# Mark-Rindler/PTRT-game-engine

Hardware: AMD Instinct MI355X
Metric: Mrays/s (higher is better)
Workload: dtype f32

## Files before the change

ptrt-game-engine_amd/csrc/pt_kernels.hip.h:

```cpp
#pragma once
#include "pt_device.hip.h"

namespace pt {

struct Camera {
    f3 origin, llc, horizontal, vertical, u, v, w;
    float lens_radius;
};

struct KParams {
    const float4 *mesh_recs;
    const float4 *nodes;
    const float4 *nodes2;
    const int2 *leaves;
    const float4 *tris;
    const int4 *slot_face;
    const float4 *tlas_nodes;
    const int2 *tlas_leaves;
    const int *tlas_mesh_ids;
    const float4 *tlas_heads;
    float inst_c2;
    const float4 *materials;
    const float4 *lights;
    const float2 *blue_noise;
    const float4 *tlas_root_box;
    int tlas_root_ref;
    int n_meshes, n_lights;
    int stack_entries;
    int pair_meshes;
    int pair_tri_slots;
    int pair_max_leaf;
    int tlas_max_leaf;
    int tlas_depth;
    int tlas_any_rounds;
    int pair_split;
    int steal;
    int csteal;
    int csteal_min;
    int csteal_follow;
    int csteal_leaf_min;
    int leaf_min;
    int leaf_pairs;
    int fetch_min;
    int n_nodes;
    int top_off;
    int n_tiles;
    int lds_extra;
    int lds_flags;
    int pair_cap;
    int lds_wave, lds_wave_bytes;
    Camera cam;
    f3 sky_top, sky_bottom;
    int use_sky;
    const float4 *env;
    int env_w, env_h;
    int width, height;
    int y0, rows;
    int il_period, il_phase;
    int tiles_x;
    int split_n, split_i;
    int spp, max_depth, frame_count;
    int sample_sync;
    int tile_run;
    uint32_t *rng;
    size_t rng_plane;
    float *accum, *normal, *depth;
    int *object_id;
    unsigned char *rgb8;
    int rgb8_frame;
    int ticket_tiles;
    unsigned int *queue;
    unsigned long long *counters;
};
constexpr int COUNTER_WORDS = 4;

PT_DEV int global_row(int yl, int y0, int il_period, int il_phase) {
    return il_period > 1 ? ((((yl >> 3) * il_period + il_phase) << 3) | (yl & 7)) : y0 + yl;
}

PT_DEV int rgb8_row(const KParams &K, int yl) {
    return K.rgb8_frame ? K.height - 1 - global_row(yl, K.y0, K.il_period, K.il_phase) : K.rows - 1 - yl;
}

constexpr int MESH_REC_F4 = 12;
constexpr int NODE2_F4 = 12;
constexpr int TOP_LEVELS = 3;
constexpr int TOP_NODES = (1 << TOP_LEVELS) - 1;
constexpr int TLAS_HEAD_F4 = 7;
// ... 713 lines not shown
```

ptrt-game-engine_amd/csrc/pt_render.hip.h:

```cpp
#pragma once
#include "pt_kernels.hip.h"

namespace pt {

struct CycleAcc;
struct PairLds {
    CycleAcc *cyc;
    int stat_bounce;
    float4 *tris;
    int4 *meshtab;
    float4 *meshbox;
    const float4 *topnodes;
    uint32_t *pairs;
    unsigned long long *best;
    uint32_t *occ;
    uint2 *stack;
    int *leafx;
    uint2 *tstack;
    unsigned long long *lkey;
    unsigned char *owner;
    const float2 *jit;
    const float2 *bn;
    const float4 *lights;
    const float4 *mats;
// ... 49 lines not shown
    char *p = (char *)base;
    const int meshes = K.pair_meshes;
    l.tris = (float4 *)p;
    p += (size_t)K.pair_tri_slots * 48 + (size_t)meshes * PAIR_PAD * 16;
    l.meshtab = (int4 *)p;
    p += (size_t)meshes * 16;
    l.meshbox = (float4 *)p;
    char *x = (char *)base + K.lds_extra;
    l.jit = (const float2 *)x;
    l.lights = (const float4 *)(x + 16 * 8);
    l.mats = l.lights + ((K.lds_flags & 1) ? K.n_lights * 4 : 0);
    char *w = (char *)base + K.lds_wave + wave * K.lds_wave_bytes;
    l.best = (unsigned long long *)w;
    l.occ = (uint32_t *)(w + 256);
    l.pairs = (uint32_t *)(w + 512);
    w += 512 + pm1_pair_bytes(meshes);
    l.bn = (const float2 *)w;
    w += (K.lds_flags & 8) ? 64 * 8 : 0;
    l.count = (unsigned long long *)w;
    return l;
}

PT_DEV size_t shared_lds_bytes(int meshes) { return (size_t)meshes * (32 + TOP_NODES * 64); }
PT_DEV size_t wave_lds_bytes(int meshes, int stack_entries) {
    return 512 + (size_t)meshes * 128 + 256 + (size_t)stack_entries * 512 + LEAF_PAIR_BYTES;
}
PT_DEV PairLds carve_pair_lds_wg(void *base, int wave, int meshes, int stack_entries) {
    PairLds l{};
    char *p = (char *)base;
    l.meshtab = nullptr;
    l.meshbox = (float4 *)p;
    p += (size_t)meshes * 32;
    l.topnodes = (const float4 *)p;
    p += (size_t)meshes * TOP_NODES * 64;
    p += (size_t)wave * wave_lds_bytes(meshes, stack_entries);
    l.best = (unsigned long long *)p;
    p += 512;
    l.pairs = (uint32_t *)p;
    p += (size_t)meshes * 128;
    l.occ = (uint32_t *)p;
    p += 256;
    l.stack = (uint2 *)p;
    p += (size_t)stack_entries * 512;
    l.lkey = (unsigned long long *)p;
    p += 512;
    l.owner = (unsigned char *)p;
    l.tris = nullptr;
    l.tstack = nullptr;
    l.leafx = nullptr;
    return l;
}

__device__ unsigned long long g_trav_bounce[64];
__device__ unsigned long long g_trav_stats[32];
#ifdef PT_MARKS
#define PT_MARK(x) asm volatile("; MARK " x)
#else
#define PT_MARK(x)
#endif
#ifdef PT_TRAV_STATS
struct TravStats {
    unsigned v[8] = {0, 0, 0, 0, 0, 0, 0, 0};
    PT_DEV void wave(int i, int lane) {
        if (lane == __builtin_ctzll(__builtin_amdgcn_ballot_w64(true)))
            ++v[i];
    }
    PT_DEV void lanes(int i) { ++v[i]; }
    PT_DEV void flush(int base, int lane, int bounce = -1) {
        for (int i = 0; i < 8; ++i) {
            unsigned a = v[i];
            for (int off = 32; off > 0; off >>= 1)
                a += __shfl_xor(a, off);
            if (lane == 0 && a) {
                atomicAdd(&g_trav_stats[base + i], (unsigned long long)a);
                if (bounce >= 0)
                    atomicAdd(&g_trav_bounce[(bounce < 3 ? bounce : 3) * 16 + base + i], (unsigned long long)a);
            }
        }
    }
};
__device__ unsigned long long g_trav_dbg[4 * 256 + 1 + 8];
#define TS_DBG(a, b, c, d)                                                                                                \
    do {                                                                                                                 \
        const unsigned long long i_ = atomicAdd(&g_trav_dbg[1024], 1ull);                                                \
        if (i_ < 256) {                                                                                                  \
            g_trav_dbg[4 * i_] = (a);                                                                                    \
            g_trav_dbg[4 * i_ + 1] = (b);                                                                                \
            g_trav_dbg[4 * i_ + 2] = (c);                                                                                \
            g_trav_dbg[4 * i_ + 3] = (d);                                                                                \
        }                                                                                                                \
    } while (0)
#define TS_EVENT(slot) atomicAdd(&g_trav_dbg[1025 + (slot)], 1ull)
#define TS_WAVE(i) ts.wave(i, lane)
#define TS_LANE(i) ts.lanes(i)
struct CycleAcc {
    unsigned long long c[8] = {0, 0, 0, 0, 0, 0, 0, 0};
    PT_DEV void flush(int lane) {
        if (lane == 0)
            for (int i = 0; i < 8; ++i)
                atomicAdd(&g_trav_stats[24 + i], c[i]);
    }
};
#define TS_LANES(slot, cond)                                                                                             \
    do {                                                                                                                 \
        const unsigned long long ts_m = __builtin_amdgcn_ballot_w64(cond);                                               \
        if (lane == __builtin_ctzll(__builtin_amdgcn_ballot_w64(true)))                                                   \
            atomicAdd(&g_trav_stats[slot], (unsigned long long)__builtin_popcountll(ts_m));                                 \
    } while (0)
#define TS_NOW() __builtin_readcyclecounter()
#define TS_ADD(slot, t) (cyc.c[(slot) - 8] += __builtin_readcyclecounter() - (t))
#define TS_ADDL(slot, t) (L.cyc->c[(slot) - 8] += __builtin_readcyclecounter() - (t))
#ifdef PT_TS_SHADING
constexpr bool TS_SHADING = true;
#else
constexpr bool TS_SHADING = false;
#endif
#define TS_ADDQ(slot, t) do { if (!TS_SHADING) TS_ADD(slot, t); } while (0)
#define TS_ADDLQ(slot, t) do { if (!TS_SHADING) TS_ADDL(slot, t); } while (0)
#else
constexpr bool TS_SHADING = false;
#define TS_ADDQ(slot, t) (void)(t)
#define TS_ADDLQ(slot, t) (void)(t)
struct TravStats {
    PT_DEV void flush(int, int, int = -1) {}
};
#define TS_EVENT(slot)
#define TS_DBG(a, b, c, d)
#define TS_WAVE(i)
#define TS_LANE(i)
struct CycleAcc {
    PT_DEV void flush(int) {}
};
#define TS_LANES(slot, cond)
#define TS_NOW() 0ull
#define TS_ADD(slot, t) (void)(t)
#define TS_ADDL(slot, t) (void)(t)
#endif

PT_DEV void wave_lds_order() {
    __builtin_amdgcn_wave_barrier();
    asm volatile("" ::: "memory");
}

PT_DEV void wave_sync() { wave_lds_order(); }

PT_DEV int lane_prefix(unsigned long long mask) {
    return __builtin_amdgcn_mbcnt_hi((uint32_t)(mask >> 32), __builtin_amdgcn_mbcnt_lo((uint32_t)mask, 0u));
}

PT_DEV MeshHead staged_mesh_head(const PairLds &L, int i) {
    const float4 a = L.meshbox[2 * i], b = L.meshbox[2 * i + 1];
    MeshHead h;
    h.bmin = mk3(a.x, a.y, a.z);
    h.bmax = mk3(b.x, b.y, b.z);
    h.root_ref = __builtin_amdgcn_readfirstlane(__float_as_int(a.w));
    const int fm = __builtin_amdgcn_readfirstlane(__float_as_int(b.w));
    h.flags = fm & 0xff;
    h.mesh = fm >> 8;
    return h;
}
PT_DEV int4 staged_mesh_entry(const PairLds &L, int i) {
    const int root = __float_as_int(lds_ld1((const float *)L.meshbox, 8 * i + 3));
    const int fm = __float_as_int(lds_ld1((const float *)L.meshbox, 8 * i + 7));
    return make_int4(root, 0, fm & 0xff, fm >> 8);
}

PT_DEV void leaf_prefix(int cnt, int &start, int &total) {
    int st = 0, tot = 0;
#pragma unroll
    for (int b = 0; b < 5; ++b) {
        const unsigned long long m = __builtin_amdgcn_ballot_w64((cnt >> b) & 1);
        st += lane_prefix(m) << b;
        tot += __builtin_popcountll(m) << b;
    }
    start = st;
    total = tot;
}

template <bool ANY>
PT_DEV int build_pairs(const KParams &K, const PairLds &L, int lane, bool alive, f3 o, f3 d, float tMax) {
    const RayO w = make_ray(o, d);
    float tE;
    alive = alive && slab(tlas_bmin(K), tlas_bmax(K), w, ANY ? tMax : T_FAR, tE);
    if (ANY)
        L.occ[lane] = 0u;
    else
        L.best[lane] = ~0ull;
    int base = 0;
    for (int i = 0; i < K.pair_meshes; ++i) {
        const MeshHead mh = staged_mesh_head(L, i);
        if (ANY && (mh.flags & 2))
            continue;
        bool hb;
        if (mh.flags & 1) {
            float ds;
            const RayO lr = local_ray(K, mh.mesh, w, ds);
            hb = alive && slab(mh.bmin, mh.bmax, lr, ANY ? tMax * ds : T_FAR, tE);
        } else {
            hb = alive && slab(mh.bmin, mh.bmax, w, ANY ? tMax : T_FAR, tE);
        }
        const unsigned long long bal = __builtin_amdgcn_ballot_w64(hb);
        if (hb) {
            ((uint16_t *)L.pairs)[base + lane_prefix(bal)] = (uint16_t)((uint32_t)lane | ((uint32_t)i << 6));
        }
        base += __builtin_popcountll(bal);
    }
    return base;
}

template <int GEN = 0> PT_DEV void pair_ray_from(const KParams &K, const int4 mt, f3 &o, f3 &d, float &dirScale) {
    dirScale = 1.0f;
    if (mt.z & 1) {
        const float4 *rec = GEN ? (K.tlas_heads + mt.w * TLAS_HEAD_F4) : (K.mesh_recs + mt.w * MESH_REC_F4);
        const f3 lo = xform_point(rec[2], rec[3], rec[4], o);
        const f3 ld = xform_dir(rec[2], rec[3], rec[4], d);
        dirScale = length(ld);
        o = lo;
        d = normalize(ld);
    }
}

PT_DEV Hit closest_hit_pairs(const KParams &K, const PairLds &L, int lane, bool alive, f3 o, f3 d, int &order) {
    const int P = build_pairs<false>(K, L, lane, alive, o, d, T_FAR);
    wave_sync();
    for (int c = 0; c < P; c += 64) {
        const int n = (P - c) < 64 ? (P - c) : 64;
        int sh = 0;
        while (K.pair_split && (n << (sh + 1)) <= 64 && (2 << sh) <= K.pair_max_leaf)
            ++sh;
        const int p = c + (lane >> sh), sub = lane & ((1 << sh) - 1);
        const bool valid = (lane >> sh) < n;
        const uint32_t e = ((const uint16_t *)L.pairs)[valid ? p : 0];
        const int r = (int)(e & 63u), oi = (int)(e >> 6);
        const int4 mt = L.meshtab[oi];
        f3 po = mk3(__shfl(o.x, r), __shfl(o.y, r), __shfl(o.z, r));
        f3 pd = mk3(__shfl(d.x, r), __shfl(d.y, r), __shfl(d.z, r));
        float dirScale;
        pair_ray_from<false>(K, mt, po, pd, dirScale);
        RayO pr;
        pr.o = po;
        pr.d = pd;
        float tb = T_FAR;
        int bi = -1;
        const int iters = (K.pair_max_leaf + (1 << sh) - 1) >> sh;
        for (int it = 0; it < iters; ++it) {
            const int i = sub + (it << sh);
            const int slot = mt.x + (i < mt.y ? i : 0);
            const float4 *tp = L.tris + slot * 3 + oi * PAIR_PAD;
            const float4 p0 = tp[0], p1 = tp[1], p2 = tp[2];
            asm volatile("" ::"v"(p0.w), "v"(p1.w), "v"(p2.w));
            float t, u, v;
            const bool ok = tri_test(mk3(p0.x, p0.y, p0.z), mk3(p1.x, p1.y, p1.z), mk3(p2.x, p2.y, p2.z), pr, tb, t, u, v);
            if (ok && i < mt.y) {
                tb = t;
                bi = i;
            }
        }
        if (valid && bi >= 0) {
            const float tw = (mt.z & 1) ? tb / dirScale : tb;
            const unsigned long long key =
                ((unsigned long long)__float_as_uint(tw) << 32) | ((unsigned long long)(uint32_t)oi << 16) | (uint32_t)bi;
            __hip_atomic_fetch_min(&L.best[r], key, __ATOMIC_RELAXED, __HIP_MEMORY_SCOPE_WORKGROUP);
        }
    }
    wave_sync();
    const unsigned long long key = L.best[lane];
    wave_sync();
    Hit h;
    h.u = h.v = 0.0f;
    order = 0;
    if (!alive || key == ~0ull) {
        h.t = h.t_local = T_FAR;
        h.mesh = -1;
        h.slot = -1;
        return h;
    }
    const int oi = (int)((key >> 16) & 0xffffu), bi = (int)(key & 0xffffu);
    order = oi;
    const int4 mt = L.meshtab[oi];
    h.t = __uint_as_float((uint32_t)(key >> 32));
    h.mesh = mt.w;
    h.slot = mt.x + bi;
    h.t_local = h.t;
    if (mt.z & 1) {
        const float4 *rec = K.mesh_recs + mt.w * MESH_REC_F4;
        RayO pr;
        pr.o = xform_point(rec[2], rec[3], rec[4], o);
        pr.d = normalize(xform_dir(rec[2], rec[3], rec[4], d));
        const float4 *tp = L.tris + h.slot * 3 + oi * PAIR_PAD;
        const float4 p0 = tp[0], p1 = tp[1], p2 = tp[2];
        float t, u, v;
        tri_test(mk3(p0.x, p0.y, p0.z), mk3(p1.x, p1.y, p1.z), mk3(p2.x, p2.y, p2.z), pr, T_FAR, t, u, v);
        h.t_local = t;
    }
    return h;
}

PT_DEV bool any_hit_pairs(const KParams &K, const PairLds &L, int lane, bool alive, f3 o, f3 d, float tMax) {
    const int P = build_pairs<true>(K, L, lane, alive, o, d, tMax);
    float *tmaxv = (float *)L.best;
    tmaxv[lane] = tMax;
    wave_sync();
    for (int c = 0; c < P; c += 64) {
        const int n = (P - c) < 64 ? (P - c) : 64;
        int sh = 0;
        while ((n << (sh + 1)) <= 64 && (2 << sh) <= K.pair_max_leaf)
            ++sh;
        const int p = c + (lane >> sh), sub = lane & ((1 << sh) - 1);
        const bool valid = (lane >> sh) < n;
        const uint32_t e = ((const uint16_t *)L.pairs)[valid ? p : 0];
        const int r = (int)(e & 63u), oi = (int)(e >> 6);
        const int4 mt = L.meshtab[oi];
        f3 po = mk3(__shfl(o.x, r), __shfl(o.y, r), __shfl(o.z, r));
        f3 pd = mk3(__shfl(d.x, r), __shfl(d.y, r), __shfl(d.z, r));
        float dirScale;
        pair_ray_from<false>(K, mt, po, pd, dirScale);
        RayO pr;
        pr.o = po;
        pr.d = pd;
        float tm = tmaxv[r];
        if (mt.z & 1)
            tm = tm * dirScale;
        bool found = false;
        const int iters = (K.pair_max_leaf + (1 << sh) - 1) >> sh;
        for (int it = 0; it < iters; ++it) {
            const int i = sub + (it << sh);
            const int slot = mt.x + (i < mt.y ? i : 0);
            const float4 *tp = L.tris + slot * 3 + oi * PAIR_PAD;
            const float4 p0 = tp[0], p1 = tp[1], p2 = tp[2];
            asm volatile("" ::"v"(p0.w), "v"(p1.w), "v"(p2.w));
            float t, u, v;
            const bool ok = tri_test(mk3(p0.x, p0.y, p0.z), mk3(p1.x, p1.y, p1.z), mk3(p2.x, p2.y, p2.z), pr, tm, t, u, v);
            found |= ok && (i < mt.y);
        }
        if (valid && found)
            L.occ[r] = 1u;
    }
    wave_sync();
    const bool occluded = alive && (L.occ[lane] != 0u);
    wave_sync();
    return occluded;
}

template <int GEN> PT_DEV int4 pair_mesh(const KParams &K, const PairLds &L, int r, int order) {
    if (!GEN)
        return staged_mesh_entry(L, order);
    const int j = GEN == 2 ? order : L.leafx[(order & (TLAS_SLOTS - 1)) * 64 + r] + (order >> 2);
    const int root = __float_as_int(K.tlas_heads[TLAS_HEAD_F4 * j].w), flags = __float_as_int(K.tlas_heads[TLAS_HEAD_F4 * j + 1].w);
    return make_int4(root, 0, flags, j);
}

PT_DEV void fetch_node(const KParams &K, const PairLds &L, int cur, int local, int order, float4 &n0, float4 &n1, float4 &n2,
                       float4 &n3) {
    if (L.topnodes && (unsigned)local < (unsigned)TOP_NODES) {
        const float4 *q = L.topnodes + (order * TOP_NODES + local) * 4;
        n0 = q[0];
        n1 = q[1];
        n2 = q[2];
        n3 = q[3];
    } else {
        n0 = K.nodes[cur * 4 + 0];
        n1 = K.nodes[cur * 4 + 1];
        n2 = K.nodes[cur * 4 + 2];
        n3 = K.nodes[cur * 4 + 3];
    }
}

#ifndef PT_TWO_LEVEL
#define PT_TWO_LEVEL 0
#endif
PT_DEV bool descend2(const float4 *__restrict__ nodes2, LdsStack stk, int &sp, const RayO &pr, float tb, int &cur) {
    const float4 *rec = nodes2 + (size_t)cur * NODE2_F4;
    const float4 n0 = rec[0], n1 = rec[1], n2 = rec[2], n3 = rec[3];
    float tL, tR;
    const bool hL = slab(mk3(n0.x, n0.y, n0.z), mk3(n0.w, n1.x, n1.y), pr, tb, tL);
    const bool hR = slab(mk3(n1.z, n1.w, n2.x), mk3(n2.y, n2.z, n2.w), pr, tb, tR);
    if (!(hL || hR))
        return true;
    const bool nearL = hL && (!hR || tL <= tR);
    const int Lr = __float_as_int(n3.x), Rr = __float_as_int(n3.y);
    if (nearL ? hR : hL) {
        stk.push(sp, nearL ? Rr : Lr, nearL ? tR : tL);
        ++sp;
    }
    cur = nearL ? Lr : Rr;
    if (cur < 0)
        return false;
    const float4 *g = rec + (nearL ? 4 : 8);
    const float4 g0 = g[0], g1 = g[1], g2 = g[2], g3 = g[3];
    const bool hGL = slab(mk3(g0.x, g0.y, g0.z), mk3(g0.w, g1.x, g1.y), pr, tb, tL);
    const bool hGR = slab(mk3(g1.z, g1.w, g2.x), mk3(g2.y, g2.z, g2.w), pr, tb, tR);
    if (!(hGL || hGR))
// ... 1299 lines not shown
                rd = normalize(dir);
            } else {
                f3 p;
                do {
                    const float a = rng_uniform(rng);
                    const float b = rng_uniform(rng);
                    p = 2.0f * mk3(a, b, 0.0f) - mk3(1.0f, 1.0f, 0.0f);
                } while (dot(p, p) >= 1.0f);
                const f3 rdisk = KA.cam.lens_radius * p;
                const f3 offset = KA.cam.u * rdisk.x + KA.cam.v * rdisk.y;
                const f3 dir = KA.cam.llc + u * KA.cam.horizontal + v * KA.cam.vertical - KA.cam.origin - offset;
                ro = KA.cam.origin + offset;
                rd = normalize(dir);
            }
            ray_spec = true;
            prev_was_specular = true;
            throughput = mk3(1.0f);
            if (!MERGED)
                acc = mk3(0.0f);
            sb &= 0xffff;
            fresh = false;
        }

        if (PMODE == 1 || TS_SHADING)
            TS_ADD(8, t_pa);
        const bool act = live && !fresh;
#ifdef PT_TRAV_STATS
        {
            const unsigned long long am = __builtin_amdgcn_ballot_w64(act);
            PL.stat_bounce = am ? __builtin_amdgcn_readlane(sb >> 16, __builtin_ctzll(am)) : -1;
        }
#endif
        PT_MARK("B");
        phase_prio<PMODE, 1, 0>();
        const KParams &KB = kparams(kp0);
        Hit h;
        int h_order = 0;
        if (MERGED) {
            bool blocked = false;
            const unsigned long long t_tr = TS_NOW();
            trace_merged(KB, PL, lane, act, ro, rd, pending, park_o, park_d, park_tmax, h, blocked, cyc);
            TS_ADD(12, t_tr);
            if (pending && !blocked)
                acc = acc + pend;
            pending = false;
            if (fin) {
                acc = clamp_vector_soft(acc, 100.0f);
                close_sample(acc);
                acc = mk3(0.0f);
                fin = false;
            }
        } else {
            const unsigned long long t_tr = TS_NOW();
            h = (PMODE == 1)   ? closest_hit_pairs(KB, PL, lane, act, ro, rd, h_order)
                : (PMODE == 2) ? closest_hit_pairs_dyn(KB, PL, lane, act, ro, rd)
                : (PMODE == 3) ? closest_hit_pairs_tlas(KB, PL, lane, act, ro, rd, cyc)
                               : closest_hit<GEOM>(KB, act, ro, rd, stk);
            TS_ADD(12, t_tr);
        }

        PT_MARK("C");
        phase_prio<PMODE, 2, 1>();
        const KParams &KC = kparams(kp0);
        const unsigned long long t_pc = TS_NOW();
        bool end_path = false, shaded = false, want_shadow = false;
        Surface hit;
        hit.point = hit.normal = mk3(0.0f);
        hit.t = 0.0f;
        hit.front_face = true;
        f3 L = mk3(0.0f), light_scale = mk3(0.0f), shadow_o = mk3(0.0f);
        float pdf_sample = 1.0f, shadow_tmax = 0.0f, light_att = 1.0f;
        if (!LDS_COUNT)
            n_ext += (uint32_t)__builtin_popcountll(__builtin_amdgcn_ballot_w64(act));
        if (act) {
            if (h.mesh < 0) {
                if (sb == 0) {
                    const size_t idx = pidx(KC.width);
                    float zero = 0.0f;
                    asm volatile("" : "+v"(zero));
                    KC.normal[idx * 3 + 0] = zero;
                    KC.normal[idx * 3 + 1] = zero;
                    KC.normal[idx * 3 + 2] = zero;
                    KC.depth[idx] = 1e30f;
                    KC.object_id[idx] = -1;
                }
                if (KC.use_sky) {
                    if (KC.env) {
                        const float phi = det_atan2(rd.z, rd.x);
                        const float theta = det_acos(max_(-1.0f, min_(1.0f, rd.y)));
                        const float u = (phi + PI_F) * (1.0f / TWO_PI_F);
                        const float v = theta * (1.0f / PI_F);
                        acc = acc + throughput * tex2d_env(KC.env, KC.env_w, KC.env_h, u, v);
                    } else {
                        const float t = 0.5f * (rd.y + 1.0f);
                        acc = acc + throughput * lerp(KC.sky_bottom, KC.sky_top, t);
                    }
                } else {
                    acc = acc + throughput * mk3(0.0f);
                }
                end_path = true;
            } else {
                shaded = true;
                if (PMODE == 1) {
                    const int ti = (h.slot * 3 + h_order * PAIR_PAD) * 4;
                    const f3 gn = mk3(lds_ld1((const float *)PL.tris, ti + 3), lds_ld1((const float *)PL.tris, ti + 7),
                                      lds_ld1((const float *)PL.tris, ti + 11));
                    const int fl = __float_as_int(lds_ld1((const float *)PL.meshtab, h_order * 4 + 2));
// ... 91 lines not shown
        PT_MARK("C2");
        phase_prio<PMODE, 3, 2>();
        const KParams &KC2 = kparams(kp0);
        const unsigned long long t_pc2 = TS_NOW();
        bool lit = false;
        f3 lit_now = mk3(0.0f);
        if (want_shadow) {
            int mi = mats_lds ? h_order : h.mesh;
            asm volatile("" : "+v"(mi));
            const Material mat = mats_lds ? load_material<true, MAT_F4>(PL.mats, mi) : load_material(KC2.materials, mi);
            const f3 V = -rd;
            const f3 bsdf = evaluateBSDF<FULL>(hit, mat, L, V);
            if (pdf_sample > 0.0f) {
                f3 direct = bsdf * light_scale * light_att / pdf_sample;
                direct = clamp_vector_soft(direct, 500.0f);
                if (direct.x > 0.0f || direct.y > 0.0f || direct.z > 0.0f) {
                    const float pdf_brdf = material_pdf<FULL>(hit, mat, V, L);
                    const float wgt = mis_weight(pdf_sample, pdf_brdf);
                    lit_now = throughput * direct * wgt;
                    lit = true;
                }
            }
        }

        {
            const unsigned long long zm = __builtin_amdgcn_ballot_w64(want_shadow && !lit);
            if (zm) {
                if (LDS_COUNT) {
                    if (lane == 0)
                        __hip_atomic_fetch_add((__attribute__((address_space(3))) unsigned long long *)(lds_count + 1),
                                               (unsigned long long)__builtin_popcountll(zm), __ATOMIC_RELAXED,
                                               __HIP_MEMORY_SCOPE_WORKGROUP);
                } else {
                    n_zero += (uint32_t)__builtin_popcountll(zm);
                }
            }
        }
        if (PMODE == 1 || TS_SHADING)
            TS_ADD(10, t_pc2);
        TS_LANES(21, lit);
        PT_MARK("D");
        phase_prio<PMODE, 4, 3>();
        const KParams &KD = kparams(kp0);
        const unsigned long long t_sh = TS_NOW();
        if (MERGED) {
            if (lit) {
                pend = lit_now;
                park_o = shadow_o;
                park_d = L;
                park_tmax = shadow_tmax;
                pending = true;
            }
        } else if (__builtin_amdgcn_ballot_w64(lit)) {
            const bool in_shadow = (PMODE == 1)   ? any_hit_pairs(KD, PL, lane, lit, shadow_o, L, shadow_tmax)
                                   : (PMODE == 2) ? any_hit_pairs_dyn(KD, PL, lane, lit, shadow_o, L, shadow_tmax)
                                   : (PMODE == 3) ? any_hit_pairs_tlas(KD, PL, lane, lit, shadow_o, L, shadow_tmax, cyc)
                                                  : any_hit<GEOM>(KD, lit, shadow_o, L, shadow_tmax, stk);
            if (lit && !in_shadow)
                acc = acc + lit_now;
        }
        TS_ADD(13, t_sh);

        PT_MARK("E");
        phase_prio<PMODE, 5, 4>();
        const KParams &KE = kparams(kp0);
        const unsigned long long t_pe = TS_NOW();
        if (shaded) {
            const Material mat = mats_lds ? load_material<true, MAT_F4>(PL.mats, h_order) : load_material(KE.materials, h.mesh);
            f3 scatter_dir = mk3(0.0f), att = mk3(0.0f);
            bool is_specular = false;
            const bool last = (sb >> 16) + 1 >= KE.max_depth;
            if (!material_scatter<FULL>(hit, mat, rd, rng, scatter_dir, att, is_specular, last)) {
                end_path = true;
            } else {
                prev_was_specular = is_specular;
                bool killed = false;
                if (sb >= 0x20000) {
                    const float p = max_(0.05f, min_(0.95f, max_(throughput.x, max_(throughput.y, throughput.z))));
                    if (rng_uniform(rng) > p)
                        killed = true;
                    else if (!last)
                        throughput = throughput / p;
                }
                if (killed || last) {
                    end_path = true;
                } else {
                    throughput = throughput * att;
                    throughput = clamp_vector_soft(throughput, 50.0f);
                    const f3 off = hit.normal * 1e-4f;
                    ro = (dot(scatter_dir, hit.normal) > 0.0f) ? (hit.point + off) : (hit.point - off);
                    rd = scatter_dir;
                    ray_spec = is_specular;
                    sb += 0x10000;
                    if ((sb >> 16) >= KE.max_depth)
                        end_path = true;
                }
            }
        }
        if (act && end_path) {
            if (MERGED && pending) {
                fin = true;
            } else {
                acc = clamp_vector_soft(acc, 100.0f);
                close_sample(acc);
                if (MERGED)
                    acc = mk3(0.0f);
            }
// ... 126 lines not shown
```

ptrt-game-engine_amd/csrc/ptrt_capi.hip:

```cpp
#include "../../include/ptrt.h"
#include "pt_build.hip.h"
#include "pt_denoise.hip.h"
#include "pt_post.hip.h"
#include "pt_refit.hip.h"
#include "pt_tlas.hip.h"
#include "pt_render.hip.h"
#include "pt_wavefront.hip.h"
#include "pt_async.hip.h"
#include "pt_wireframe.hip.h"
#include "pt_query.hip.h"
#include "rt_render.hip.h"

#include <hip/hip_runtime.h>

#include <cmath>
#include <cstdarg>
#include <cstdio>
#include <climits>
#include <cstring>
#include <map>
#include <mutex>
#include <set>
#include <string>
#include <algorithm>
// ... 87 lines not shown
    int use_graphs = 0;
    bool tlas_single_leaf = false, all_single_leaf = false, mats_full = false;
    int stack_entries = 1;
    int pair_meshes = 0, pair_tri_slots = 0, pair_max_leaf = 0;
    int tlas_max_leaf = 0, tlas_depth = 0;
    bool have_geometry = false, have_materials = false;

    pt::Camera cam{};
    pt::f3 sky_top{0.6f, 0.7f, 1.0f}, sky_bottom{1.0f, 1.0f, 1.0f};
    int use_sky = 1;
    float4 *d_env = nullptr;
    int env_w = 0, env_h = 0;

    bool dn_on = false, dn_first = true;
    pt::DenoiseSettings dn{};
    float4 *dn_cur4 = nullptr, *dn_c4[2] = {nullptr, nullptr}, *dn_g4[2] = {nullptr, nullptr};
    float4 *dn_h1[2] = {nullptr, nullptr}, *dn_h2[2] = {nullptr, nullptr};
    int *dn_hobj = nullptr;
    float *dn_motion = nullptr, *dn_out = nullptr, *dn_pvp = nullptr;
    int dn_cur = 0;
    int dn_active = 1, mv_active = 1;
    float prev_view_proj[16] = {1, 0, 0, 0, 0, 1, 0, 0, 0, 0, 1, 0, 0, 0, 0, 1};

    int rw = 0, rh = 0;
    float *s_accum = nullptr, *s_normal = nullptr, *s_depth = nullptr;
    int *s_object_id = nullptr;
    int bloom_on = 0;
    float *bl_mip[6] = {nullptr, nullptr, nullptr, nullptr, nullptr, nullptr};
    bool scaled() const { return rw != W || rh != H; }
    size_t rpix() const { return scaled() ? (size_t)rw * rh : npix; }

    FrameRing present;

    int wavefront = 0;
    int wf_sort = 0;
    uint32_t *wf_st = nullptr, *wf_occ = nullptr, *wf_live = nullptr;
    float *wf_planes = nullptr;
    float4 *wf_hit = nullptr;
    size_t wf_items = 0;
    int wf_trace_blocks = 0;
    size_t wf_trace_lds = 0;
    int n_geometry_uploads = 0, n_instance_updates = 0;
    bool any_transform = false;
    int pair_split = 1;
    int last_mode = 0;
    int async_lanes = 0, shade_min = 32, as_leaf_min = 24;
    uint32_t *as_cursor = nullptr;
    int refill = 1;
    bool refill_eff = false;
    VertexStage verts;
    unsigned int *d_queue = nullptr;
    int sample_sync = -1;
    int sample_sync_eff = 0;
    int tile_run = 8;
    int ticket_tiles = 1;
    int persist = 0, n_cus = 0;
    int as_blocks[2] = {0, 0};
    size_t as_lds = 0;

    int count_rays = 0, force_geom = -1, force_full = 0, pair_trace = 1, fetch_min = 16, leaf_pairs = 1, steal = 1, leaf_min = 8;
    int atrous_exp = 0;
    int csteal_follow = 1, csteal_leaf_min = 32;
    int csteal = 2, csteal_min = 0;
    int lds_pad = 0;
    int pm1_wg = 1;
    static constexpr int MAX_SPLIT = 4;
    int split = 2, split_eff = 1, pipeline = 1;
    hipStream_t aux_stream[MAX_SPLIT] = {nullptr, nullptr, nullptr, nullptr};
    hipEvent_t split_fork = nullptr, split_join[MAX_SPLIT] = {nullptr, nullptr, nullptr, nullptr};
    bool heads_fresh = false;
    bool touched = true;
    bool escaped = false;
    void *prev_out = nullptr;
    hipStream_t prev_stream = nullptr;
    int prev_split = 0;
    bool pipelined_last = false;
    hipEvent_t head_ev[2] = {nullptr, nullptr};
    unsigned head_n = 0;
    int tlas_rounds = 0;
    int stage = 7;
    int lds_nodes = 0;
    int n_nodes = 0;
    int merged = -1;
    int merged_eff = 0;
    int tune_n = 0, tune_choice = -1;
    unsigned long long tune_key = ~0ull, tune_launch[2 * TUNE_SAMPLES] = {};
    int last_pmode = 0;
    int query_pmode = -1;
    bool last_merged_possible = false;
    bool timed = false;
    bool prev_post = false;
    size_t refill_counter_base = 0;
    int time_launches = 0;
    std::vector<hipEvent_t> launch_ev[MAX_SPLIT];
    unsigned char launch_timed[EV_RING] = {};
    int tm_prio = 0;
    hipStream_t tm_stream[MAX_SPLIT] = {nullptr, nullptr, nullptr, nullptr};
    hipEvent_t tm_fork[MAX_SPLIT] = {nullptr, nullptr, nullptr, nullptr}, tm_join[MAX_SPLIT] = {nullptr, nullptr, nullptr, nullptr};
};

namespace {

int fail(ptrt_ctx *c, int code, const char *fmt, ...) {
    char buf[512];
    va_list ap;
    va_start(ap, fmt);
// ... 1255 lines not shown
    } else if (splittable && c->last_mode == 0) {
        if (!c->split_fork)
            HIP_TRY(c, hipEventCreateWithFlags(&c->split_fork, hipEventDisableTiming));
        HIP_TRY(c, hipEventRecord(c->split_fork, c->stream));
        c->prev_split = 1;
    }
    return PTRT_OK;
}

}

extern "C" {

int ptrt_render(ptrt_ctx *c, int frame_index, int spp, int max_depth, void *out_rgb8, int out_is_device) {
    if (!ctx_live(c, false))
        return fail(c, PTRT_E_INVALID, "ptrt_render: bad context");
    if (!c->have_geometry || !c->have_materials)
        return fail(c, PTRT_E_NOT_READY, "ptrt_render: %s not uploaded", c->have_geometry ? "materials" : "geometry");
    if (c->n_materials < c->n_meshes)
        return fail(c, PTRT_E_NOT_READY, "ptrt_render: %d materials for %d meshes", c->n_materials, c->n_meshes);
    if (!c->rng_ready)
        return fail(c, PTRT_E_NOT_READY, "ptrt_render: generator states not initialised (ptrt_reset_rng)");
    if (spp < 1 || max_depth < 1 || spp > 32767 || max_depth > 32767)
        return fail(c, PTRT_E_INVALID, "ptrt_render: spp=%d max_depth=%d (1..32767)", spp, max_depth);
    if (frame_index < 0 || frame_index > INT_MAX - spp)
        return fail(c, PTRT_E_INVALID, "ptrt_render: frame_index=%d", frame_index);
    if (int rc = set_device(c))
        return rc;
    pt::KParams K = make_params(c);
    K.spp = spp;
    K.max_depth = max_depth;
    K.sample_sync = c->sample_sync >= 0 ? c->sample_sync : (max_depth <= 4 ? 1 : 0);
    c->sample_sync_eff = K.sample_sync;
    K.tile_run = c->tile_run;
    K.frame_count = frame_index;
    unsigned char *frame_rgb8 = (out_rgb8 && out_is_device) ? (unsigned char *)out_rgb8 : c->d_rgb8;
    const bool scaled = c->scaled(), denoise = c->dn_on && c->dn_active, bloom = c->bloom_on != 0;
    const bool into_frame = out_rgb8 && out_is_device == PTRT_OUT_DEVICE_FRAME;
    if (into_frame && (denoise || bloom || scaled))
        return fail(c, PTRT_E_INVALID, "ptrt_render: PTRT_OUT_DEVICE_FRAME with the denoiser, bloom or a reduced render size");
    c->last_rgb8 = into_frame ? nullptr : frame_rgb8;
    c->last_frame_target = into_frame ? out_rgb8 : nullptr;
    K.rgb8_frame = into_frame ? 1 : 0;
    K.rgb8 = (denoise || bloom || scaled) ? nullptr : frame_rgb8;
    if (c->count_rays)
        K.counters = c->d_counters;
    const int tiles_y = (K.rows + 7) / 8;
    const int grid = K.tiles_x * tiles_y;
    const int geom = pick_geom(c);
    const bool full = c->mats_full || c->force_full;
    const bool tuning = choose_loop_shape(c, spp, max_depth, geom);
    const int pmode = pair_mode(c, geom, c->merged_eff != 0);
    c->last_pmode = pmode;
    if (c->merged < 0 && pmode == 4 && c->csteal == 0)
        K.steal = 0;
    const size_t lds = pmode ? pair_lds_bytes(c, pmode) : ((geom == 0) ? 0 : (size_t)c->stack_entries * 64 * sizeof(uint2));
    if (pmode == 3 && (c->touched || !c->heads_fresh)) {
        c->heads_fresh = true;
        hipLaunchKernelGGL(pt::gather_tlas_heads_kernel, dim3((c->n_tlas_index + 63) / 64), dim3(64), 0, c->stream,
                           c->d_mesh_recs, c->d_inst_pre, c->d_tlas_mesh_ids, c->n_tlas_index, c->d_tlas_heads,
                           c->inst_pre_ok ? 1 : 0);
        HIP_TRY(c, hipGetLastError());
    }
    size_t lds_main = lds + (size_t)c->lds_pad;
    int pm1_wg = 1;
    if (pmode == 1)
        lds_main = pm1_layout(c, K, full, grid, pm1_wg);
    if (c->launches == 0 && getenv("PTRT_DEBUG_LDS"))
        fprintf(stderr, "ptrt: pmode %d, %d meshes in the leaf, %d triangle slots, stack %d, LDS %zu + %zu bytes per workgroup\n", pmode,
                c->pair_meshes, c->pair_tri_slots, c->stack_entries, lds, lds_main - lds);
    const int slot = (int)(c->launches % EV_RING);
    const bool timing = c->time_kernels || tuning;
    if (timing)
        HIP_TRY(c, hipEventRecord(c->ev_ring[2 * slot], c->stream));
    const bool post = denoise || bloom;
    OverlapPlan plan;
    if (int rc = plan_overlap(c, K, spp, max_depth, pmode, pm1_wg, tiles_y, tuning, scaled, post, out_rgb8, out_is_device, plan))
        return rc;
    const long per_launch = (long)grid / (c->split_eff > 1 ? c->split_eff : 1);
    const long resident = (long)c->n_cus * (c->persist > 0 ? c->persist : 4 * pt::waves_per_simd(1, full, 1));
    c->refill_eff = pmode == 1 && pm1_wg == 1 &&
                    (c->refill == 2 || (c->refill == 1 && c->pipelined_last && !full && !denoise && !bloom &&
                                        (long)spp * max_depth >= 16 && per_launch >= 2 * resident));
    c->prev_out = (out_rgb8 && out_is_device) ? out_rgb8 : nullptr;
    c->prev_stream = c->stream;
    c->touched = false;
    c->last_mode = 0;
    c->launch_timed[slot] = 0;
    if (int rc = launch_frame(c, K, full, spp, max_depth, geom, pmode, pm1_wg, grid, lds, lds_main))
        return rc;
    if (int rc = join_frame(c, plan, post))
        return rc;
    if (timing)
        HIP_TRY(c, hipEventRecord(c->ev_ring[2 * slot + 1], c->stream));
    if (tuning) {
        if (c->tune_n >= TUNE_WARM)
            c->tune_launch[c->tune_n - TUNE_WARM] = c->launches;
        ++c->tune_n;
    }
    c->launches++;
    c->timed = timing;
    float *current = K.accum;
    if (denoise) {
        if (int rc = run_denoiser(c, K, (bloom || scaled) ? nullptr : frame_rgb8))
            return rc;
        current = c->dn_out;
// ... 718 lines not shown
```

ptrt-game-engine_amd/csrc/ptrt_options.hip.h:

```cpp
#pragma once

namespace {

template <class Launch> int run_check(ptrt_ctx *c, unsigned int *out9, Launch launch) {
    if (int rc = set_device(c))
        return rc;
    DeviceTemp<unsigned int> d;
    HIP_TRY(c, d.alloc(9));
    HIP_TRY(c, hipMemset(d.p, 0, 9 * sizeof(unsigned int)));
    launch(d.p);
    HIP_TRY(c, hipStreamSynchronize(c->stream));
    HIP_TRY(c, hipMemcpy(out9, d.p, 9 * sizeof(unsigned int), hipMemcpyDeviceToHost));
    return PTRT_OK;
}

enum OptPolicy {
    OPT_READ_ONLY,
    OPT_BOOL,
    OPT_REJECT,
    OPT_CLAMP,
    OPT_MASK,
    OPT_TRISTATE,
    OPT_SNAP_124,
};

struct Option {
    const char *name;
    int ptrt_ctx::*field;
    OptPolicy policy;
    long long lo, hi;
    long long (*get)(const ptrt_ctx *);
    void (*set)(ptrt_ctx *, int);
};

const Option OPTIONS[] = {
    {"count_rays", &ptrt_ctx::count_rays, OPT_BOOL},
    {"force_geom", &ptrt_ctx::force_geom, OPT_REJECT, -1, 2},
    {"force_full", &ptrt_ctx::force_full, OPT_BOOL},
    {"pair_trace", &ptrt_ctx::pair_trace, OPT_BOOL},
    {"steal", &ptrt_ctx::steal, OPT_REJECT, 0, 64},
    {"csteal", &ptrt_ctx::csteal, OPT_REJECT, 0, 64},
    {"atrous_exp", &ptrt_ctx::atrous_exp, OPT_BOOL},
    {"csteal_follow", &ptrt_ctx::csteal_follow, OPT_BOOL},
    {"csteal_leaf_min", &ptrt_ctx::csteal_leaf_min, OPT_REJECT, 1, 64},
    {"csteal_min", &ptrt_ctx::csteal_min, OPT_REJECT, 0, 1024},
    {"lds_nodes", &ptrt_ctx::lds_nodes, OPT_CLAMP, 0, 2},
    {"merged", &ptrt_ctx::merged, OPT_TRISTATE},
    {"leaf_pairs", &ptrt_ctx::leaf_pairs, OPT_BOOL},
    {"lds_pad", &ptrt_ctx::lds_pad, OPT_REJECT, 0, 32768},
    {"time_kernels", &ptrt_ctx::time_kernels, OPT_BOOL},
    {"time_launches", &ptrt_ctx::time_launches, OPT_BOOL},
    {"tm_prio", &ptrt_ctx::tm_prio, OPT_MASK, 0, 3},
    {"pipeline", &ptrt_ctx::pipeline, OPT_BOOL},
    {"persist", &ptrt_ctx::persist, OPT_CLAMP, 0, INT_MAX},
    {"sample_sync", &ptrt_ctx::sample_sync, OPT_TRISTATE},
    {"tile_run", &ptrt_ctx::tile_run, OPT_REJECT, 0, 64},
    {"ticket_tiles", &ptrt_ctx::ticket_tiles, OPT_CLAMP, 1, 16},
    {"refill", &ptrt_ctx::refill, OPT_CLAMP, 0, 2},
    {"split", &ptrt_ctx::split, OPT_REJECT, 1, ptrt_ctx::MAX_SPLIT},
    {"tlas_rounds", &ptrt_ctx::tlas_rounds, OPT_BOOL},
    {"pm1_wg", &ptrt_ctx::pm1_wg, OPT_REJECT, 0, 2},
    {"stage", &ptrt_ctx::stage, OPT_MASK, 0, 7},
    {"pair_split", &ptrt_ctx::pair_split, OPT_BOOL},
    {"async_lanes", &ptrt_ctx::async_lanes, OPT_BOOL},
    {"shade_min", &ptrt_ctx::shade_min, OPT_REJECT, 1, 64},
    {"leaf_min", &ptrt_ctx::leaf_min, OPT_REJECT, 1, 64, nullptr, [](ptrt_ctx *c, int v) { c->leaf_min = c->as_leaf_min = v; }},
    {"wavefront", &ptrt_ctx::wavefront, OPT_BOOL},
    {"wf_sort", &ptrt_ctx::wf_sort, OPT_SNAP_124},
    {"fetch_min", &ptrt_ctx::fetch_min, OPT_REJECT, 0, 64},
    {"denoiser_active", &ptrt_ctx::dn_active, OPT_BOOL},
    {"motion_vectors", &ptrt_ctx::mv_active, OPT_BOOL},
    {"use_graphs", &ptrt_ctx::use_graphs, OPT_BOOL},
    {"sample_sync_eff", &ptrt_ctx::sample_sync_eff, OPT_READ_ONLY},
    {"refilled", nullptr, OPT_READ_ONLY, 0, 0, [](const ptrt_ctx *c) -> long long { return c->refill_eff ? 1 : 0; }},
    {"split_eff", &ptrt_ctx::split_eff, OPT_READ_ONLY},
    {"pipelined", nullptr, OPT_READ_ONLY, 0, 0, [](const ptrt_ctx *c) -> long long { return c->pipelined_last ? 1 : 0; }},
    {"render_mode", &ptrt_ctx::last_mode, OPT_READ_ONLY},
    {"pmode", &ptrt_ctx::last_pmode, OPT_READ_ONLY},
    {"merged_eff", &ptrt_ctx::merged_eff, OPT_READ_ONLY},
    {"merged_decided", nullptr, OPT_READ_ONLY, 0, 0,
     [](const ptrt_ctx *c) -> long long { return (c->merged >= 0 || c->tune_choice >= 0 || !c->last_merged_possible) ? 1 : 0; }},
    {"launches", nullptr, OPT_READ_ONLY, 0, 0, [](const ptrt_ctx *c) { return (long long)c->launches; }},
    {"query_pmode", &ptrt_ctx::query_pmode, OPT_READ_ONLY},
    {"inst_pre_ok", nullptr, OPT_READ_ONLY, 0, 0, [](const ptrt_ctx *c) -> long long { return c->inst_pre_ok ? 1 : 0; }},
    {"tlas_refits", &ptrt_ctx::tlas_refits, OPT_READ_ONLY},
    {"tlas_reorders", &ptrt_ctx::tlas_reorders, OPT_READ_ONLY},
    {"stream", nullptr, OPT_READ_ONLY, 0, 0, [](const ptrt_ctx *c) { return (long long)(intptr_t)c->stream; }},
};

const Option *find_option(const char *name) {
    for (const Option &o : OPTIONS)
        if (std::strcmp(o.name, name) == 0)
            return &o;
    return nullptr;
}

}

extern "C" {

int ptrt_set_option(ptrt_ctx *c, const char *name, long long value) {
    if (!ctx_live(c, false) || !name)
        return fail(c, PTRT_E_INVALID, "ptrt_set_option: bad argument");
    const Option *o = find_option(name);
    if (!o || o->policy == OPT_READ_ONLY)
        return fail(c, PTRT_E_INVALID, "unknown option '%s'", name);
    long long v = value;
    switch (o->policy) {
    case OPT_BOOL: v = value ? 1 : 0; break;
    case OPT_REJECT:
        if (value < o->lo || value > o->hi)
            return fail(c, PTRT_E_INVALID, "%s must be %lld..%lld", name, o->lo, o->hi);
        break;
    case OPT_CLAMP: v = value < o->lo ? o->lo : (value > o->hi ? o->hi : value); break;
    case OPT_MASK: v = value & o->hi; break;
    case OPT_TRISTATE: v = value < 0 ? -1 : (value ? 1 : 0); break;
    case OPT_SNAP_124: v = value <= 0 ? 0 : (value >= 4 ? 4 : (value >= 2 ? 2 : 1)); break;
    case OPT_READ_ONLY: break;
    }
    if (o->set)
        o->set(c, (int)v);
    else
        c->*(o->field) = (int)v;
    return PTRT_OK;
}

int ptrt_get_option(ptrt_ctx *c, const char *name, long long *value) {
    if (!ctx_live(c, false) || !name || !value)
        return fail(c, PTRT_E_INVALID, "ptrt_get_option: bad argument");
    const Option *o = find_option(name);
    if (!o)
        return fail(c, PTRT_E_INVALID, "unknown option '%s'", name);
    *value = o->get ? o->get(c) : c->*(o->field);
    return PTRT_OK;
}

int ptrt_debug_last_render_mode(ptrt_ctx *c) { return ctx_live(c) ? c->last_mode : -1; }

int ptrt_debug_trav_stats(ptrt_ctx *c, unsigned long long *out32) {
    if (!ctx_live(c) || !out32)
        return fail(c, PTRT_E_INVALID, "ptrt_debug_trav_stats: bad argument");
    if (int rc = set_device(c))
        return rc;
    HIP_TRY(c, hipStreamSynchronize(c->stream));
    HIP_TRY(c, hipMemcpyFromSymbol(out32, HIP_SYMBOL(pt::g_trav_stats), 32 * sizeof(unsigned long long)));
    unsigned long long zero[32] = {};
    HIP_TRY(c, hipMemcpyToSymbol(HIP_SYMBOL(pt::g_trav_stats), zero, sizeof(zero)));
    return PTRT_OK;
}

int ptrt_debug_trav_bounce(ptrt_ctx *c, unsigned long long *out64) {
    if (!ctx_live(c) || !out64)
        return fail(c, PTRT_E_INVALID, "ptrt_debug_trav_bounce: bad argument");
    if (int rc = set_device(c))
        return rc;
    HIP_TRY(c, hipStreamSynchronize(c->stream));
    HIP_TRY(c, hipMemcpyFromSymbol(out64, HIP_SYMBOL(pt::g_trav_bounce), 64 * sizeof(unsigned long long)));
    unsigned long long zero[64] = {};
    HIP_TRY(c, hipMemcpyToSymbol(HIP_SYMBOL(pt::g_trav_bounce), zero, sizeof(zero)));
    return PTRT_OK;
}

#ifdef PT_TRAV_STATS
int ptrt_debug_trav_dbg(ptrt_ctx *c, unsigned long long *out1033) {
    if (!ctx_live(c) || !out1033)
        return fail(c, PTRT_E_INVALID, "ptrt_debug_trav_dbg: bad argument");
    HIP_TRY(c, hipStreamSynchronize(c->stream));
    HIP_TRY(c, hipMemcpyFromSymbol(out1033, HIP_SYMBOL(pt::g_trav_dbg), 1033 * sizeof(unsigned long long)));
    static unsigned long long zero[1033] = {};
    HIP_TRY(c, hipMemcpyToSymbol(HIP_SYMBOL(pt::g_trav_dbg), zero, sizeof(zero)));
    return PTRT_OK;
}
#endif

int ptrt_debug_rcp_check(ptrt_ctx *c, unsigned int *out9) {
    if (!ctx_live(c) || !out9)
        return fail(c, PTRT_E_INVALID, "ptrt_debug_rcp_check: bad argument");
    return run_check(c, out9, [c](unsigned int *d) { hipLaunchKernelGGL(pt::rcp_check_kernel, dim3(4096), dim3(256), 0, c->stream, d); });
}

int ptrt_debug_sqrt_check(ptrt_ctx *c, unsigned int *out9) {
    if (!ctx_live(c) || !out9)
        return fail(c, PTRT_E_INVALID, "ptrt_debug_sqrt_check: bad argument");
    return run_check(c, out9, [c](unsigned int *d) { hipLaunchKernelGGL(pt::sqrt_check_kernel, dim3(4096), dim3(256), 0, c->stream, d); });
}

int ptrt_debug_div3_check(ptrt_ctx *c, unsigned int first, unsigned int count, int mode, unsigned int *out9) {
    if (!ctx_live(c) || !out9 || count == 0 || count > (1u << 23) || mode < 0 || mode > 3)
        return fail(c, PTRT_E_INVALID, "ptrt_debug_div3_check: bad argument");
    return run_check(c, out9, [=](unsigned int *d) {
        hipLaunchKernelGGL(pt::div3_check_kernel, dim3((count + 63) / 64), dim3(64), 0, c->stream, first, count, mode, d);
    });
}

int ptrt_debug_detmath(ptrt_ctx *c, int op, const float *x, const float *y, int n, float *out) {
    if (!ctx_live(c) || !x || !out || n <= 0)
        return fail(c, PTRT_E_INVALID, "ptrt_debug_detmath: bad argument");
    if (int rc = set_device(c))
        return rc;
    DeviceTemp<float> dx, dy, dout;
    HIP_TRY(c, dx.alloc((size_t)n));
    HIP_TRY(c, dy.alloc((size_t)n));
    HIP_TRY(c, dout.alloc((size_t)n));
    HIP_TRY(c, hipMemcpy(dx.p, x, (size_t)n * 4, hipMemcpyHostToDevice));
    HIP_TRY(c, hipMemcpy(dy.p, y ? y : x, (size_t)n * 4, hipMemcpyHostToDevice));
    hipLaunchKernelGGL(pt::detmath_kernel, dim3((n + 255) / 256), dim3(256), 0, c->stream, op, dx.p, dy.p, n, dout.p);
    HIP_TRY(c, hipStreamSynchronize(c->stream));
    HIP_TRY(c, hipMemcpy(out, dout.p, (size_t)n * 4, hipMemcpyDeviceToHost));
    return PTRT_OK;
}

int ptrt_debug_shade(ptrt_ctx *c, int op, int full, const float *in, int n, float *out) {
    if (!ctx_live(c) || !in || !out || n <= 0 || (op != 0 && op != 1))
        return fail(c, PTRT_E_INVALID, "ptrt_debug_shade: bad argument");
    if (!c->have_materials)
        return fail(c, PTRT_E_NOT_READY, "ptrt_debug_shade: materials not uploaded");
// ... 18 lines not shown
```

Before: 27260.

## Compact live rays and spread mesh-box tests across lanes in pair building

Adds a dense path for pair building in pair mode 1. When at most 32 lanes of a wave hold live rays, those rays are compacted into LDS and replicated across lane groups, so each group tests a different subset of mesh boxes per iteration. This replaces the old loop, where every lane tested every mesh, in order to cut idle-lane work when few rays survive the TLAS root test. It costs extra shuffles, an LDS owner table and a separate handling branch for transformed meshes, and it is enabled by default only when there are at least 4 pair meshes.

```diff
diff --git a/ptrt-game-engine_amd/csrc/pt_kernels.hip.h b/ptrt-game-engine_amd/csrc/pt_kernels.hip.h
--- a/ptrt-game-engine_amd/csrc/pt_kernels.hip.h
+++ b/ptrt-game-engine_amd/csrc/pt_kernels.hip.h
@@ -34,6 +34,7 @@
     int tlas_depth;
     int tlas_any_rounds;
     int pair_split;
+    int pm1_dense;
     int steal;
     int csteal;
     int csteal_min;
diff --git a/ptrt-game-engine_amd/csrc/pt_render.hip.h b/ptrt-game-engine_amd/csrc/pt_render.hip.h
--- a/ptrt-game-engine_amd/csrc/pt_render.hip.h
+++ b/ptrt-game-engine_amd/csrc/pt_render.hip.h
@@ -125,6 +125,7 @@
 }
 
 __device__ unsigned long long g_trav_bounce[64];
+__device__ unsigned long long g_trav_rhist[8];
 __device__ unsigned long long g_trav_stats[32];
 #ifdef PT_MARKS
 #define PT_MARK(x) asm volatile("; MARK " x)
@@ -179,6 +180,12 @@
         const unsigned long long ts_m = __builtin_amdgcn_ballot_w64(cond);                                               \
         if (lane == __builtin_ctzll(__builtin_amdgcn_ballot_w64(true)))                                                   \
             atomicAdd(&g_trav_stats[slot], (unsigned long long)__builtin_popcountll(ts_m));                                 \
+    } while (0)
+#define TS_RHIST(any, cond)                                                                                              \
+    do {                                                                                                                 \
+        const int ts_r = __builtin_popcountll(__builtin_amdgcn_ballot_w64(cond));                                        \
+        if (lane == __builtin_ctzll(__builtin_amdgcn_ballot_w64(true)))                                                   \
+            atomicAdd(&g_trav_rhist[((any) ? 4 : 0) + (ts_r == 0 ? 0 : ts_r <= 16 ? 1 : ts_r <= 32 ? 2 : 3)], 1ull);       \
     } while (0)
 #define TS_NOW() __builtin_readcyclecounter()
 #define TS_ADD(slot, t) (cyc.c[(slot) - 8] += __builtin_readcyclecounter() - (t))
@@ -205,6 +212,7 @@
     PT_DEV void flush(int) {}
 };
 #define TS_LANES(slot, cond)
+#define TS_RHIST(any, cond)
 #define TS_NOW() 0ull
 #define TS_ADD(slot, t) (void)(t)
 #define TS_ADDL(slot, t) (void)(t)
@@ -251,14 +259,79 @@
 }
 
 template <bool ANY>
+PT_DEV int build_pairs_dense(const KParams &K, const PairLds &L, int lane, bool alive, unsigned long long lm, int R, const RayO &w,
+                             float tMax) {
+    const int M = K.pair_meshes;
+    unsigned char *own = (unsigned char *)L.pairs + 64 * M;
+    if (alive)
+        own[lane_prefix(lm)] = (unsigned char)lane;
+    wave_sync();
+    const int wsh = R <= 16 ? 4 : 5;
+    const int rk = lane & ((1 << wsh) - 1), G = 64 >> wsh;
+    const bool has = rk < R;
+    uint32_t e = (uint32_t)(has ? (int)own[rk] : lane) | ((uint32_t)(lane >> wsh) << 6);
+    RayO q;
+    q.o = mk3(__shfl(w.o.x, (int)(e & 63u)), __shfl(w.o.y, (int)(e & 63u)), __shfl(w.o.z, (int)(e & 63u)));
+    q.inv = mk3(__shfl(w.inv.x, (int)(e & 63u)), __shfl(w.inv.y, (int)(e & 63u)), __shfl(w.inv.z, (int)(e & 63u)));
+    q.d = q.inv;
+    q.sx = q.inv.x < 0;
+    q.sy = q.inv.y < 0;
+    q.sz = q.inv.z < 0;
+    const float tm = ANY ? __shfl(tMax, (int)(e & 63u)) : T_FAR;
+    int base = 0;
+    for (int i0 = 0; i0 < M; i0 += G, e += (uint32_t)G << 6) {
+        const int i = (int)(e >> 6);
+        const float *hp = (const float *)L.meshbox + 8 * (i < M ? i : 0);
+        const int fm = __float_as_int(lds_ld1(hp, 7));
+        const bool cand = has && i < M && !(ANY && (fm & 2));
+        const bool xf = cand && (fm & 1);
+        float tE;
+        bool hb = cand && !xf &&
+                  slab(mk3(lds_ld1(hp, 0), lds_ld1(hp, 1), lds_ld1(hp, 2)), mk3(lds_ld1(hp, 4), lds_ld1(hp, 5), lds_ld1(hp, 6)), q, tm, tE);
+        if (__builtin_amdgcn_ballot_w64(xf)) {
+            RayO wr = q;
+            wr.d = mk3(__shfl(w.d.x, (int)(e & 63u)), __shfl(w.d.y, (int)(e & 63u)), __shfl(w.d.z, (int)(e & 63u)));
+            if (xf) {
+                float ds;
+                const RayO lr = local_ray(K, fm >> 8, wr, ds);
+                wave_lds_order();
+                hb = slab(mk3(lds_ld1(hp, 0), lds_ld1(hp, 1), lds_ld1(hp, 2)), mk3(lds_ld1(hp, 4), lds_ld1(hp, 5), lds_ld1(hp, 6)), lr,
+                          ANY ? tm * ds : T_FAR, tE);
+            }
+        }
+        const unsigned long long bal = __builtin_amdgcn_ballot_w64(hb);
+        if (hb) {
+            ((uint16_t *)L.pairs)[base + lane_prefix(bal)] = (uint16_t)e;
+        }
+        base += __builtin_popcountll(bal);
+    }
+    return base;
+}
+
+PT_DEV int lane_here(int lane) {
+    int z = 0;
+    asm volatile("" : "+s"(z));
+    return lane + z;
+}
+
+template <bool ANY, bool DENSE = false>
 PT_DEV int build_pairs(const KParams &K, const PairLds &L, int lane, bool alive, f3 o, f3 d, float tMax) {
     const RayO w = make_ray(o, d);
     float tE;
     alive = alive && slab(tlas_bmin(K), tlas_bmax(K), w, ANY ? tMax : T_FAR, tE);
     if (ANY)
-        L.occ[lane] = 0u;
+        L.occ[DENSE ? lane_here(lane) : lane] = 0u;
     else
         L.best[lane] = ~0ull;
+    TS_RHIST(ANY, alive);
+    if (DENSE && K.pm1_dense) {
+        const unsigned long long lm = __builtin_amdgcn_ballot_w64(alive);
+        const int R = __builtin_popcountll(lm);
+        if (R == 0)
+            return 0;
+        if (R <= 32)
+            return build_pairs_dense<ANY>(K, L, lane, alive, lm, R, w, tMax);
+    }
     int base = 0;
     for (int i = 0; i < K.pair_meshes; ++i) {
         const MeshHead mh = staged_mesh_head(L, i);
@@ -293,8 +366,9 @@
     }
 }
 
+template <bool DENSE = false>
 PT_DEV Hit closest_hit_pairs(const KParams &K, const PairLds &L, int lane, bool alive, f3 o, f3 d, int &order) {
-    const int P = build_pairs<false>(K, L, lane, alive, o, d, T_FAR);
+    const int P = build_pairs<false, DENSE>(K, L, lane, alive, o, d, T_FAR);
     wave_sync();
     for (int c = 0; c < P; c += 64) {
         const int n = (P - c) < 64 ? (P - c) : 64;
@@ -369,10 +443,11 @@
     return h;
 }
 
+template <bool DENSE = false>
 PT_DEV bool any_hit_pairs(const KParams &K, const PairLds &L, int lane, bool alive, f3 o, f3 d, float tMax) {
-    const int P = build_pairs<true>(K, L, lane, alive, o, d, tMax);
     float *tmaxv = (float *)L.best;
-    tmaxv[lane] = tMax;
+    tmaxv[DENSE ? lane_here(lane) : lane] = tMax;
+    const int P = build_pairs<true, DENSE>(K, L, lane, alive, o, d, tMax);
     wave_sync();
     for (int c = 0; c < P; c += 64) {
         const int n = (P - c) < 64 ? (P - c) : 64;
@@ -410,7 +485,7 @@
             L.occ[r] = 1u;
     }
     wave_sync();
-    const bool occluded = alive && (L.occ[lane] != 0u);
+    const bool occluded = alive && (L.occ[DENSE ? lane_here(lane) : lane] != 0u);
     wave_sync();
     return occluded;
 }
@@ -1816,7 +1891,7 @@
             }
         } else {
             const unsigned long long t_tr = TS_NOW();
-            h = (PMODE == 1)   ? closest_hit_pairs(KB, PL, lane, act, ro, rd, h_order)
+            h = (PMODE == 1)   ? closest_hit_pairs<true>(KB, PL, lane, act, ro, rd, h_order)
                 : (PMODE == 2) ? closest_hit_pairs_dyn(KB, PL, lane, act, ro, rd)
                 : (PMODE == 3) ? closest_hit_pairs_tlas(KB, PL, lane, act, ro, rd, cyc)
                                : closest_hit<GEOM>(KB, act, ro, rd, stk);
@@ -2014,7 +2089,7 @@
                 pending = true;
             }
         } else if (__builtin_amdgcn_ballot_w64(lit)) {
-            const bool in_shadow = (PMODE == 1)   ? any_hit_pairs(KD, PL, lane, lit, shadow_o, L, shadow_tmax)
+            const bool in_shadow = (PMODE == 1)   ? any_hit_pairs<true>(KD, PL, lane, lit, shadow_o, L, shadow_tmax)
                                    : (PMODE == 2) ? any_hit_pairs_dyn(KD, PL, lane, lit, shadow_o, L, shadow_tmax)
                                    : (PMODE == 3) ? any_hit_pairs_tlas(KD, PL, lane, lit, shadow_o, L, shadow_tmax, cyc)
                                                   : any_hit<GEOM>(KD, lit, shadow_o, L, shadow_tmax, stk);
diff --git a/ptrt-game-engine_amd/csrc/ptrt_capi.hip b/ptrt-game-engine_amd/csrc/ptrt_capi.hip
--- a/ptrt-game-engine_amd/csrc/ptrt_capi.hip
+++ b/ptrt-game-engine_amd/csrc/ptrt_capi.hip
@@ -163,6 +163,8 @@
     unsigned int *d_queue = nullptr;
     int sample_sync = -1;
     int sample_sync_eff = 0;
+    int pm1_dense_roots = -1;
+    int pm1_dense_roots_eff = 0;
     int tile_run = 8;
     int ticket_tiles = 1;
     int persist = 0, n_cus = 0;
@@ -1524,6 +1526,8 @@
     const bool tuning = choose_loop_shape(c, spp, max_depth, geom);
     const int pmode = pair_mode(c, geom, c->merged_eff != 0);
     c->last_pmode = pmode;
+    K.pm1_dense = (pmode == 1 && (c->pm1_dense_roots >= 0 ? c->pm1_dense_roots : (c->pair_meshes >= 4 ? 1 : 0))) ? 1 : 0;
+    c->pm1_dense_roots_eff = K.pm1_dense;
     if (c->merged < 0 && pmode == 4 && c->csteal == 0)
         K.steal = 0;
     const size_t lds = pmode ? pair_lds_bytes(c, pmode) : ((geom == 0) ? 0 : (size_t)c->stack_entries * 64 * sizeof(uint2));
diff --git a/ptrt-game-engine_amd/csrc/ptrt_options.hip.h b/ptrt-game-engine_amd/csrc/ptrt_options.hip.h
--- a/ptrt-game-engine_amd/csrc/ptrt_options.hip.h
+++ b/ptrt-game-engine_amd/csrc/ptrt_options.hip.h
@@ -54,6 +54,7 @@
     {"pipeline", &ptrt_ctx::pipeline, OPT_BOOL},
     {"persist", &ptrt_ctx::persist, OPT_CLAMP, 0, INT_MAX},
     {"sample_sync", &ptrt_ctx::sample_sync, OPT_TRISTATE},
+    {"pm1_dense_roots", &ptrt_ctx::pm1_dense_roots, OPT_TRISTATE},
     {"tile_run", &ptrt_ctx::tile_run, OPT_REJECT, 0, 64},
     {"ticket_tiles", &ptrt_ctx::ticket_tiles, OPT_CLAMP, 1, 16},
     {"refill", &ptrt_ctx::refill, OPT_CLAMP, 0, 2},
@@ -72,6 +73,7 @@
     {"motion_vectors", &ptrt_ctx::mv_active, OPT_BOOL},
     {"use_graphs", &ptrt_ctx::use_graphs, OPT_BOOL},
     {"sample_sync_eff", &ptrt_ctx::sample_sync_eff, OPT_READ_ONLY},
+    {"pm1_dense_roots_eff", &ptrt_ctx::pm1_dense_roots_eff, OPT_READ_ONLY},
     {"refilled", nullptr, OPT_READ_ONLY, 0, 0, [](const ptrt_ctx *c) -> long long { return c->refill_eff ? 1 : 0; }},
     {"split_eff", &ptrt_ctx::split_eff, OPT_READ_ONLY},
     {"pipelined", nullptr, OPT_READ_ONLY, 0, 0, [](const ptrt_ctx *c) -> long long { return c->pipelined_last ? 1 : 0; }},
@@ -162,6 +164,16 @@
 }
 
 #ifdef PT_TRAV_STATS
+int ptrt_debug_trav_rhist(ptrt_ctx *c, unsigned long long *out8) {
+    if (!ctx_live(c) || !out8)
+        return fail(c, PTRT_E_INVALID, "ptrt_debug_trav_rhist: bad argument");
+    HIP_TRY(c, hipStreamSynchronize(c->stream));
+    HIP_TRY(c, hipMemcpyFromSymbol(out8, HIP_SYMBOL(pt::g_trav_rhist), 8 * sizeof(unsigned long long)));
+    unsigned long long zero[8] = {};
+    HIP_TRY(c, hipMemcpyToSymbol(HIP_SYMBOL(pt::g_trav_rhist), zero, sizeof(zero)));
+    return PTRT_OK;
+}
+
 int ptrt_debug_trav_dbg(ptrt_ctx *c, unsigned long long *out1033) {
     if (!ctx_live(c) || !out1033)
         return fail(c, PTRT_E_INVALID, "ptrt_debug_trav_dbg: bad argument");
```

New measurement: 27900 (median of 6 runs). 1.02x the previous value.
